# PolusAI/nyxus

Measured on AMD Instinct MI355X. Metric: ROIs/sec (*ALL_GLCM*+*ALL_INTENSITY*, 1024^2 tiles), higher is better.
Workload: dtype f64; 1 GPU; *ALL_GLCM*+*ALL_INTENSITY*, coarse_gray_depth=8, 4 angles, d=1, 1000 synthetic 1024x1024 tiles/GPU x 196 ROIs/tile (disk r=30, 2821 px, bbox 61x61), intensities U[1,4095]; reduce stage on pre-assembled ROI clouds resident in HBM; n_columns=185

## Files before the change

### nyxus_amd/csrc/roi_features.hip

```cpp
#include <hip/hip_runtime.h>
#include <type_traits>
#include <algorithm>
#include <cstdio>
#include "knobs.h"
#include "device_math.h"
#include "roi_kernel.h"
#include "launch_util.h"
#include "glcm_rows.h"
#include "glcm_w64.h"
#include "intensity_close.h"
#include "sort_lds.h"
#include "../../include/nyxhip.h"

namespace nyxhip {


enum { S_MEAN = 0, S_P10, S_P90, S_MEDIAN, S_MODE, S_NG, S_SLOPE };


template <int NW> __device__ __forceinline__ double xw_chain(const double* s_red, int k)
{
    return NW == 1 ? s_red[k] : ((s_red[k] + s_red[8 + k]) + s_red[16 + k]) + s_red[24 + k];
}
template <int NW> __device__ __forceinline__ double xw_pairs(const double* s_red, int k)
// ... 101 lines not shown
        for (int j = 0; j < Ng; j++, ic += (uint32_t)Ng) {
            cc += P[ic];
            rc += P[lN + (uint32_t)j];
        }
        uint32_t i1 = lN, i2 = (uint32_t)l;
#pragma unroll 1
        for (int x = l; x < Ng; x++, i1 += (uint32_t)Ng + 1u, i2 += (uint32_t)Ng + 1u) {
            dc += P[i1];
            if (l > 0)
                dc += P[i2];
        }
    }
    const uint32_t l1 = (uint32_t)l + 1u;
    const uint32_t csum = row16_sum(rc);
    const uint32_t Sr_i = row16_sum(mul24(rc, l1)), Sc_i = row16_sum(mul24(cc, l1));
    const uint32_t con_i = row16_sum(mul24(dc, (uint32_t)(l * l))), dis_i = row16_sum(mul24(dc, (uint32_t)l));
    const bool empty = csum == 0;
    const double sum_p = empty ? 1.0 : (double)csum;
    const double inv_sum_p = fdiv(1.0, sum_p);
    const double mr = fdiv((double)Sr_i, sum_p), mc = fdiv((double)Sc_i, sum_p);
    const double pcol = fdiv((double)cc, sum_p), prow = fdiv((double)rc, sum_p), pxmy = fdiv((double)dc, sum_p);
    if (live && l < Ng) { pcol_s[l] = pcol; prow_s[l] = prow; }
    for (int k = l; k < 2 * Ng - 1; k += 16) {
        uint32_t c = 0;
        const int x0 = k - (Ng - 1) > 0 ? k - (Ng - 1) : 0, x1 = k < Ng - 1 ? k : Ng - 1;
        uint32_t ix = mad24((uint32_t)x0, (uint32_t)Ng, (uint32_t)(k - x0));
#pragma unroll 1
        for (int x = x0; x <= x1; x++, ix += (uint32_t)Ng - 1u)
            c += P[ix];
        if (live) Pxpy[k] = fdiv((double)c, sum_p);
    }
    wav_sync<false>();

    double ent = 0, hxy1 = 0, hxy2 = 0, asm_d = 0;
    uint32_t acor_i = 0, asm_i = 0, cmax = 0;
    const bool big = csum >= 65536u;
    RowCol rcw((uint32_t)l, 16u, (uint32_t)Ng, RowCol::small_t{});
    for (int e = l; e < NN; e += 16, rcw.advance()) {
        const uint32_t r = rcw.row, c = rcw.col, cnt = P[e];
        const double p = (double)cnt * inv_sum_p;
        if (big) asm_d = __builtin_fma(p, p, asm_d);
        else asm_i = mad24(cnt, cnt, asm_i);
        acor_i = mad24(cnt, mul24(r + 1u, c + 1u), acor_i);
        cmax = cnt > cmax ? cnt : cmax;
        ent = __builtin_fma(p, (double)fast_log2f(p + 0.000000001), ent);
        const double pp = pcol_s[c] * prow_s[r];
        const double lg = (double)fast_log2f(pp + 0.000000001);
        hxy1 = __builtin_fma(p, lg, hxy1);
        hxy2 = __builtin_fma(pp, lg, hxy2);
    }
    const double hx_t = l < Ng ? plogp(pcol, pcol) : 0.0;
    {
        double t4[4] = {ent, hxy1, hxy2, hx_t};
        transpose_sum_step<0x140, 2>(t4, (l & 8) != 0);
        transpose_sum_step<0x141, 1>(t4, (l & 4) != 0);
        double tot = t4[0];
        tot += dpp_perm<0x4E>(tot);
        tot += dpp_perm<0xB1>(tot);
        if (live && (l & 3) == 0) sm[1 + (l >> 2)] = tot;
    }
    acor_i = row16_sum(acor_i);
    asm_i = row16_sum(asm_i);
    if (big) asm_d = row16_sum(asm_d);
    {
        uint32_t o;
        o = dpp_perm<0xB1>(cmax); cmax = o > cmax ? o : cmax;
        o = dpp_perm<0x4E>(cmax); cmax = o > cmax ? o : cmax;
        o = dpp_perm<0x141>(cmax); cmax = o > cmax ? o : cmax;
        o = dpp_perm<0x140>(cmax); cmax = o > cmax ? o : cmax;
    }

    double t16[16];
#pragma unroll
    for (int k = 0; k < 16; k++) t16[k] = 0.0;
    if (l < Ng) {
        const double dr = (double)l1 - mr, dcl = (double)l1 - mc, dr2 = dr * dr;
        t16[0] = prow * dr2;
        t16[1] = pcol * (dcl * dcl);
        t16[2] = (double)rc * dr2;
        t16[3] = pcol * dr2;
        const double q = pxmy, kd = (double)l, Ngd = (double)Ng;
        t16[4] = fdiv(q, (double)(1 + l * l));
        t16[5] = q != 0 ? plogp(q, q) : 0.0;
        t16[6] = fdiv(q, 1.0 + fdiv(kd * kd, Ngd * Ngd));
        t16[7] = fdiv(q, 1.0 + kd);
        t16[8] = fdiv(q, 1.0 + fdiv(kd, Ngd));
        t16[9] = l >= 1 ? q / (kd * kd) : 0.0;
        t16[10] = kd * q;
    }
    for (int k = l; k < 2 * Ng - 1; k += 16) {
        const double q = Pxpy[k], ks = (double)(k + 2);
        t16[11] += ks * q;
        t16[12] += plogp(q, q);
        const double m = ks - mc - mc, m2 = m * m;
        t16[13] += m2 * m2 * q;
        t16[14] += m2 * m * q;
        t16[15] += m2 * q;
    }
    {
        const double tot = row16_transpose_sum16(t16, l);
        if (live) sm[8 + l] = tot;
    }
    wav_sync<false>();
    const double davg = sm[8 + 10];
    double dv = 0;
    if (l < Ng) { const double dk = (double)l - davg; dv = dk * dk * pxmy; }
    dv = row16_sum(dv);

    if (live && l == 0) {
        const double ent_t = sm[1], hxy1_t = sm[2], hxy2_t = sm[3], hx = sm[4];
        const double asm_t = big ? asm_d : (double)asm_i * inv_sum_p * inv_sum_p;
        const double cov_t = ((double)acor_i * sum_p - (double)Sr_i * (double)Sc_i) * (inv_sum_p * inv_sum_p);
        f[G_ASM] = asm_t;
        f[G_ENERGY] = asm_t;
        f[G_CONTRAST] = (double)con_i * inv_sum_p;
        f[G_ACOR] = (double)acor_i * inv_sum_p;
        f[G_ENTROPY] = -ent_t;
        f[G_JE] = -ent_t;
        f[G_DIS] = (double)dis_i * inv_sum_p;
        f[G_JMAX] = (double)cmax * inv_sum_p;
        f[G_JAVE] = mr;
        f[G_VARIANCE] = sm[8 + 2] * inv_sum_p;
        f[G_CLUPROM] = sm[8 + 13];
        f[G_CLUSHADE] = sm[8 + 14];
        f[G_CLUTEND] = sm[8 + 15];
        f[G_SUMVARIANCE] = sm[8 + 15];
        f[G_JVAR] = sm[8 + 3];
        const double vv = sm[8 + 0] * sm[8 + 1];
        f[G_CORRELATION] = !(sm[8 + 0] > 0.0 && sm[8 + 1] > 0.0) ? soft_nan : cov_t * frsq(vv);
        f[G_INFOMEAS2] = sqrt(fabs(1 - exp(-2 * (-hxy2_t + ent_t))));
        f[G_IDM] = sm[8 + 4];
        f[G_HOM2] = sm[8 + 4];
        f[G_HOM1] = sm[8 + 7];
        f[G_SUMAVERAGE] = sm[8 + 11];
        f[G_SUMENTROPY] = -sm[8 + 12];
        f[G_DIFENTRO] = -sm[8 + 5];
        f[G_DIFAVE] = davg;
        f[G_DIFVAR] = dv;
        f[G_IDMN] = sm[8 + 6];
        f[G_ID] = sm[8 + 7];
        f[G_IDN] = sm[8 + 8];
        f[G_IV] = sm[8 + 9];
        const double r1 = (ent_t - hxy1_t) / hx;
        f[G_INFOMEAS1] = isfinite(r1) ? r1 : soft_nan;
        if (empty)
            for (int k = 0; k < kGlcmAngled; k++)
                f[k] = soft_nan;
    }
    wav_sync<false>();
}

__device__ __forceinline__ uint32_t grp8_sum(uint32_t v) { v += dpp_perm<0xB1>(v); v += dpp_perm<0x4E>(v); v += dpp_perm<0x141>(v); return v; }
__device__ __forceinline__ double grp8_sum(double v) { v += dpp_perm<0xB1>(v); v += dpp_perm<0x4E>(v); v += dpp_perm<0x141>(v); return v; }
__device__ __forceinline__ void glcm_features_wave8(const uint32_t* P_a, const uint32_t* P_b, int n_slots, int Ng_a, int Ng_b, double* scr_base, int scr_stride,
                                                    double soft_nan, double* fslots, size_t f_gap, double* sums, int lane)
{
    const int grp = lane >> 3, l = lane & 7, sel = grp >> 2, slot_raw = grp & 3;
    const int Ng = sel ? Ng_b : Ng_a;
    const int NN = Ng * Ng;
    const bool live = slot_raw < n_slots && Ng != 0;
    const int slot = slot_raw < n_slots ? slot_raw : 0;
    const uint32_t* P = (sel ? P_b : P_a) + mul24((uint32_t)slot, (uint32_t)NN);
    const int gslot = sel * kMaxAngles + slot;
    double* pcol_s = scr_base + mul24((uint32_t)gslot, (uint32_t)scr_stride);
    double* prow_s = pcol_s + 8;
    double* f = fslots + gslot * 32 + (sel ? f_gap : 0);
    double* sm = sums + gslot * 32;

    uint32_t cc = 0, rc = 0, dc = 0;
    if (l < Ng) {
        const uint32_t lN = mul24((uint32_t)l, (uint32_t)Ng);
        uint32_t ic = (uint32_t)l;
#pragma unroll 1
        for (int j = 0; j < Ng; j++, ic += (uint32_t)Ng) {
            cc += P[ic];
            rc += P[lN + (uint32_t)j];
        }
        uint32_t i1 = lN, i2 = (uint32_t)l;
#pragma unroll 1
        for (int x = l; x < Ng; x++, i1 += (uint32_t)Ng + 1u, i2 += (uint32_t)Ng + 1u) {
            dc += P[i1];
            if (l > 0) dc += P[i2];
        }
    }
    const uint32_t l1 = (uint32_t)l + 1u;
    const uint32_t csum = grp8_sum(rc);
    const uint32_t Sr_i = grp8_sum(mul24(rc, l1)), Sc_i = grp8_sum(mul24(cc, l1));
    const uint32_t con_i = grp8_sum(mul24(dc, (uint32_t)(l * l))), dis_i = grp8_sum(mul24(dc, (uint32_t)l));
    const bool empty = csum == 0;
    const double sum_p = empty ? 1.0 : (double)csum;
    const double inv_sum_p = fdiv(1.0, sum_p);
    const double mr = fdiv((double)Sr_i, sum_p), mc = fdiv((double)Sc_i, sum_p);
    const double pcol = fdiv((double)cc, sum_p), prow = fdiv((double)rc, sum_p), pxmy = fdiv((double)dc, sum_p);
    if (live && l < Ng) { pcol_s[l] = pcol; prow_s[l] = prow; }
    double pxpy[2] = {0.0, 0.0};
#pragma unroll
    for (int u = 0; u < 2; u++) {
        const int k = l + 8 * u;
        if (k < 2 * Ng - 1) {
            uint32_t c = 0;
            const int x0 = k - (Ng - 1) > 0 ? k - (Ng - 1) : 0, x1 = k < Ng - 1 ? k : Ng - 1;
            uint32_t ix = mad24((uint32_t)x0, (uint32_t)Ng, (uint32_t)(k - x0));
#pragma unroll 1
            for (int x = x0; x <= x1; x++, ix += (uint32_t)Ng - 1u) c += P[ix];
            pxpy[u] = fdiv((double)c, sum_p);
        }
    }
    wav_sync<false>();
#if defined(NYX_G8_EXIT) && NYX_G8_EXIT == 1
    if (live && l < Ng) f[l] = pcol + prow + pxmy + pxpy[0] + pxpy[1] + mr + mc + (double)(con_i + dis_i);
    return;
#endif

    double ent = 0, hxy1 = 0, hxy2 = 0, asm_d = 0;
    uint32_t acor_i = 0, asm_i = 0, cmax = 0;
    const bool big = csum >= 65536u;
    {
        RowCol rcw((uint32_t)l, 8u, (uint32_t)(Ng ? Ng : 1), RowCol::small_t{});
        for (int e = l; e < NN; e += 8, rcw.advance()) {
            const uint32_t r = rcw.row, c = rcw.col, cnt = P[e];
            const double p = (double)cnt * inv_sum_p;
            if (big) asm_d = __builtin_fma(p, p, asm_d);
            else asm_i = mad24(cnt, cnt, asm_i);
            acor_i = mad24(cnt, mul24(r + 1u, c + 1u), acor_i);
            cmax = cnt > cmax ? cnt : cmax;
            ent = __builtin_fma(p, (double)fast_log2f(p + 0.000000001), ent);
            const double pp = pcol_s[c] * prow_s[r];
            const double lg = (double)fast_log2f(pp + 0.000000001);
            hxy1 = __builtin_fma(p, lg, hxy1);
            hxy2 = __builtin_fma(pp, lg, hxy2);
        }
    }
#if defined(NYX_G8_EXIT) && NYX_G8_EXIT == 2
    if (live && l < Ng) f[l] = ent + hxy1 + hxy2 + asm_d + (double)(acor_i + asm_i + cmax);
    return;
#endif
    const double hx_t = l < Ng ? plogp(pcol, pcol) : 0.0;
    {
        double t4[4] = {ent, hxy1, hxy2, hx_t};
        transpose_sum_step<0x141, 2>(t4, (l & 4) != 0);
        transpose_sum_step<0x4E, 1>(t4, (l & 2) != 0);
        double tot = t4[0];
        tot += dpp_perm<0xB1>(tot);
        if (live && (l & 1) == 0) sm[1 + (l >> 1)] = tot;
    }
    acor_i = grp8_sum(acor_i);
    asm_i = grp8_sum(asm_i);
    if (big) asm_d = grp8_sum(asm_d);
    {
        uint32_t o;
        o = dpp_perm<0xB1>(cmax); cmax = o > cmax ? o : cmax;
        o = dpp_perm<0x4E>(cmax); cmax = o > cmax ? o : cmax;
        o = dpp_perm<0x141>(cmax); cmax = o > cmax ? o : cmax;
    }

    {
        double t8[8];
#pragma unroll
        for (int k = 0; k < 8; k++) t8[k] = 0.0;
        if (l < Ng) {
            const double dr = (double)l1 - mr, dcl = (double)l1 - mc, dr2 = dr * dr;
            t8[0] = prow * dr2;
            t8[1] = pcol * (dcl * dcl);
            t8[2] = (double)rc * dr2;
            t8[3] = pcol * dr2;
            const double q = pxmy, kd = (double)l, Ngd = (double)Ng;
            t8[4] = fdiv(q, (double)(1 + l * l));
            t8[5] = q != 0 ? plogp(q, q) : 0.0;
            t8[6] = fdiv(q, 1.0 + fdiv(kd * kd, Ngd * Ngd));
            t8[7] = fdiv(q, 1.0 + kd);
        }
        transpose_sum_step<0x141, 4>(t8, (l & 4) != 0);
        transpose_sum_step<0x4E, 2>(t8, (l & 2) != 0);
        transpose_sum_step<0xB1, 1>(t8, (l & 1) != 0);
        if (live) sm[8 + l] = t8[0];
    }
    {
        double t8[8];
#pragma unroll
        for (int k = 0; k < 8; k++) t8[k] = 0.0;
        if (l < Ng) {
            const double q = pxmy, kd = (double)l, Ngd = (double)Ng;
            t8[0] = fdiv(q, 1.0 + fdiv(kd, Ngd));
            t8[1] = l >= 1 ? q / (kd * kd) : 0.0;
            t8[2] = kd * q;
        }
#pragma unroll
        for (int u = 0; u < 2; u++) {
            const int k = l + 8 * u;
            if (k < 2 * Ng - 1) {
                const double q = pxpy[u], ks = (double)(k + 2);
                t8[3] += ks * q;
                t8[4] += plogp(q, q);
                const double m = ks - mc - mc, m2 = m * m;
                t8[5] += m2 * m2 * q;
                t8[6] += m2 * m * q;
                t8[7] += m2 * q;
            }
        }
        transpose_sum_step<0x141, 4>(t8, (l & 4) != 0);
        transpose_sum_step<0x4E, 2>(t8, (l & 2) != 0);
        transpose_sum_step<0xB1, 1>(t8, (l & 1) != 0);
        if (live) sm[16 + l] = t8[0];
    }
    wav_sync<false>();
#if defined(NYX_G8_EXIT) && NYX_G8_EXIT == 3
    return;
#endif
    const double davg = sm[8 + 10];
    double dv = 0;
    if (l < Ng) { const double dk = (double)l - davg; dv = dk * dk * pxmy; }
    dv = grp8_sum(dv);

    if (live && l == 0) {
        const double ent_t = sm[1], hxy1_t = sm[2], hxy2_t = sm[3], hx = sm[4];
        const double asm_t = big ? asm_d : (double)asm_i * inv_sum_p * inv_sum_p;
        const double cov_t = ((double)acor_i * sum_p - (double)Sr_i * (double)Sc_i) * (inv_sum_p * inv_sum_p);
        f[G_ASM] = asm_t;
        f[G_ENERGY] = asm_t;
        f[G_CONTRAST] = (double)con_i * inv_sum_p;
        f[G_ACOR] = (double)acor_i * inv_sum_p;
        f[G_ENTROPY] = -ent_t;
        f[G_JE] = -ent_t;
        f[G_DIS] = (double)dis_i * inv_sum_p;
        f[G_JMAX] = (double)cmax * inv_sum_p;
        f[G_JAVE] = mr;
        f[G_VARIANCE] = sm[8 + 2] * inv_sum_p;
        f[G_CLUPROM] = sm[8 + 13];
        f[G_CLUSHADE] = sm[8 + 14];
        f[G_CLUTEND] = sm[8 + 15];
        f[G_SUMVARIANCE] = sm[8 + 15];
        f[G_JVAR] = sm[8 + 3];
        const double vv = sm[8 + 0] * sm[8 + 1];
        f[G_CORRELATION] = !(sm[8 + 0] > 0.0 && sm[8 + 1] > 0.0) ? soft_nan : cov_t * frsq(vv);
        f[G_INFOMEAS2] = sqrt(fabs(1 - exp(-2 * (-hxy2_t + ent_t))));
        f[G_IDM] = sm[8 + 4];
        f[G_HOM2] = sm[8 + 4];
        f[G_HOM1] = sm[8 + 7];
        f[G_SUMAVERAGE] = sm[8 + 11];
        f[G_SUMENTROPY] = -sm[8 + 12];
        f[G_DIFENTRO] = -sm[8 + 5];
        f[G_DIFAVE] = davg;
        f[G_DIFVAR] = dv;
        f[G_IDMN] = sm[8 + 6];
        f[G_ID] = sm[8 + 7];
        f[G_IDN] = sm[8 + 8];
        f[G_IV] = sm[8 + 9];
        const double r1 = (ent_t - hxy1_t) / hx;
        f[G_INFOMEAS1] = isfinite(r1) ? r1 : soft_nan;
        if (empty)
            for (int k = 0; k < kGlcmAngled; k++) f[k] = soft_nan;
    }
    wav_sync<false>();
}

typedef unsigned short us2_t __attribute__((ext_vector_type(2)));
#ifdef NYX_G16_EXIT
#define G16_EXIT(k, keep) do { if ((k) == NYX_G16_EXIT) { ((double*)blk)[lane & 31] = (double)(keep); return; } } while (0)
#else
#define G16_EXIT(k, keep) do { } while (0)
#endif
template <int NG, int ROLE = 0>
__device__ __forceinline__ void glcm_features_wave64_v2(const uint16_t* P, int Ng_rt, uint32_t* blk, double soft_nan, int lane)
{
    const int Ng = NG ? NG : Ng_rt;
    typedef __attribute__((address_space(3))) const uint16_t lds_cu16_t;
    typedef __attribute__((address_space(3))) const uint32_t lds_cu32_t;
    typedef __attribute__((address_space(3))) uint32_t lds_u32_t;
    const int pitch = (Ng + 3) & ~1;
    double* const f = (double*)blk;
// ... 1924 lines not shown
                for (; a < na; a++)
                    init = init + s_f[a * 32 + k];
                o[kGlcmAngled * na + j] = na ? init / (double)na : 0.0;
            }
        }
    }

    STAMP(13);
    STAMP(14);
}

template <bool GS, bool C16, bool SPLIT, bool D8>
__global__ __launch_bounds__(kBlock, 4) void roi_features_kernel(const RoiArgs A)
{
    roi_features_body<GS, C16, SPLIT, D8>(A, blockIdx.x);
}

template <bool C16, bool SPLIT, bool D8>
__global__ __launch_bounds__(kBlock, 5) void roi_features_kernel_occ5(const RoiArgs A)
{
    roi_features_body<false, C16, SPLIT, D8, 0, 5>(A, blockIdx.x);
}
template <bool C16, bool SPLIT, bool D8>
__global__ __launch_bounds__(kBlock, 6) void roi_features_kernel_occ6(const RoiArgs A)
{
    roi_features_body<false, C16, SPLIT, D8, 0, 6>(A, blockIdx.x);
}
template <bool C16, bool SPLIT, bool D8>
__global__ __launch_bounds__(kBlock, 7) void roi_features_kernel_occ7(const RoiArgs A)
{
    roi_features_body<false, C16, SPLIT, D8, 0, 7>(A, blockIdx.x);
}
template <int FAM, int WIN>
__global__ __launch_bounds__(kBlock, 8) void roi_features_kernel_occ8(const RoiArgs A)
{
    roi_features_body<false, true, FAM == 1 || FAM == 3, true, FAM, 8, false, WIN, 4, FAM == 1 || FAM == 2>(A, (WIN == 1 && A.win.xcd_swz) ? xcd_slot(blockIdx.x, gridDim.x) : (uint64_t)blockIdx.x);
}
template <int FAM, int WIN>
__global__ __launch_bounds__(kBlock, 7) void roi_features_kernel_fam7(const RoiArgs A)
{
    roi_features_body<false, true, FAM == 1 || FAM == 3, true, FAM, 7, false, WIN>(A, (WIN == 1 && A.win.xcd_swz) ? xcd_slot(blockIdx.x, gridDim.x) : (uint64_t)blockIdx.x);
}
template <int FAM, int WIN>
__global__ __launch_bounds__(kBlock, 6) void roi_features_kernel_fam6(const RoiArgs A)
{
    roi_features_body<false, true, FAM == 1 || FAM == 3, true, FAM, 6, false, WIN>(A, (WIN == 1 && A.win.xcd_swz) ? xcd_slot(blockIdx.x, gridDim.x) : (uint64_t)blockIdx.x);
}

template <int WIN>
__global__ __launch_bounds__(kBlock, 4) void roi_features_kernel_g16(const RoiArgs A)
{
    roi_features_body<false, true, false, true, 0, 9, true, WIN>(A, (WIN == 1 && A.win.xcd_swz) ? xcd_slot(blockIdx.x, gridDim.x) : (uint64_t)blockIdx.x);
}

template <int WIN>
__global__ __launch_bounds__(512, 8) void roi_features_kernel_g16w8(const RoiArgs A)
{
    roi_features_body<false, true, false, true, 4, 9, true, WIN, 8>(A, (WIN == 1 && A.win.xcd_swz) ? xcd_slot(blockIdx.x, gridDim.x) : (uint64_t)blockIdx.x);
}

__device__ __forceinline__ bool glcm_roi_in_launch(const RoiArgs& A, uint64_t roi)
{
    if (A.sp.class_mask == 0) return true;
    return roi_in_launch(A.sp, (uint32_t)(A.px_offset[roi + 1] - A.px_offset[roi]), A.bbox_w[roi], A.bbox_h[roi], A.max_inten[roi] - A.min_inten[roi]);
}

__global__ __launch_bounds__(kBlock, 4) void glcm_features_kernel(const RoiArgs A)
{
    extern __shared__ __attribute__((aligned(16))) unsigned char lds_raw[];
    const int tid = threadIdx.x, lane = tid & 63, wave = __builtin_amdgcn_readfirstlane(tid >> 6);
    uint64_t roi;
    if (!roi_of_slot(A.sp, (uint64_t)blockIdx.x * kWaves + wave, A.n_roi, roi))
        return;
    const int Ng = glcm_roi_in_launch(A, roi) ? (int)A.glcm_ng[roi] : 0;
    if (Ng == 0)
        return;
    const int na = A.glcm_na, ngc = (int)A.L.ng_cap, NN = Ng * Ng;
    const size_t per_wave = (((size_t)4 * kMaxAngles * ngc * ngc + 15) & ~(size_t)15) + 8ull * (ngc + kMaxAngles * 6 * ngc + 2 * kMaxAngles * 32);
    unsigned char* base = lds_raw + (size_t)wave * per_wave;
    uint32_t* s_P = (uint32_t*)base;
    double* s_scr = (double*)(base + (((size_t)4 * kMaxAngles * ngc * ngc + 15) & ~(size_t)15)) + ngc;
    double* s_f = s_scr + kMaxAngles * 6 * ngc;
    const uint32_t* src = A.glcm_ws + roi * A.glcm_ws_stride;
    const int nw = na * NN;
    if (((nw | (int)A.glcm_ws_stride) & 3) == 0) {
#pragma unroll 1
        for (int i = lane; i < (nw >> 2); i += 64) ((uint4*)s_P)[i] = ((const uint4*)src)[i];
    } else {
#pragma unroll 1
        for (int i = lane; i < nw; i += 64) s_P[i] = src[i];
    }
    wav_sync<false>();
    glcm_features_wave16(s_P, na, Ng, s_scr, 6 * ngc, A.soft_nan, s_f, s_f + kMaxAngles * 32, lane);
    wav_sync<false>();
    double* o = A.out + roi * A.ld + A.col_glcm;
    const int sh = na == 4 ? 2 : na == 2 ? 1 : na == 1 ? 0 : -1;
    for (int c = lane; c < kGlcmAngled * na; c += 64) {
        const int k = sh >= 0 ? c >> sh : c / na, a = c - k * na;
        o[c] = s_f[a * 32 + k];
    }
    for (int j = lane; j < kGlcmAve; j += 64) {
        const int k = c_glcm_ave_order[j];
        double init = 0.0;
        int a = 0;
        for (; na - a >= 4; a += 4) {
            const double v1 = s_f[a * 32 + k] + s_f[(a + 1) * 32 + k];
            const double v2 = s_f[(a + 2) * 32 + k] + s_f[(a + 3) * 32 + k];
            init = init + (v1 + v2);
        }
        for (; a < na; a++)
            init = init + s_f[a * 32 + k];
        o[kGlcmAngled * na + j] = na == 4 ? init * 0.25 : na == 2 ? init * 0.5 : na ? init / (double)na : 0.0;
    }
}

__host__ __device__ inline size_t glcm8_cnt_bytes(uint32_t ngc)
{
    const size_t c = ((size_t)4 * kMaxAngles * ngc * ngc + 15) & ~(size_t)15, fbytes = 8ull * kMaxAngles * 32;
    return c > fbytes ? c : fbytes;
}
__global__ __launch_bounds__(kBlock, 8) void glcm_features_kernel8(const RoiArgs A)
{
    extern __shared__ __attribute__((aligned(16))) unsigned char lds_raw[];
    const int tid = threadIdx.x, lane = tid & 63, wave = __builtin_amdgcn_readfirstlane(tid >> 6);
    const uint64_t slot0 = ((uint64_t)blockIdx.x * kWaves + wave) * 2;
    uint64_t roi[2] = {0, 0};
    int Ng[2] = {0, 0};
#pragma unroll
    for (int q = 0; q < 2; q++)
        if (roi_of_slot(A.sp, slot0 + q, A.n_roi, roi[q]) && glcm_roi_in_launch(A, roi[q])) Ng[q] = (int)A.glcm_ng[roi[q]];
    if (Ng[0] == 0 && Ng[1] == 0)
        return;
    const int na = A.glcm_na, ngc = (int)A.L.ng_cap;
    const size_t cnt_bytes = glcm8_cnt_bytes((uint32_t)ngc);
    const size_t per_wave = 2 * cnt_bytes + 8ull * (2 * kMaxAngles * 16 + 2 * kMaxAngles * 32);
    unsigned char* base = lds_raw + (size_t)wave * per_wave;
    uint32_t* s_P[2] = {(uint32_t*)base, (uint32_t*)(base + cnt_bytes)};
    double* s_scr = (double*)(base + 2 * cnt_bytes);
    double* s_sum = s_scr + 2 * kMaxAngles * 16;
#pragma unroll
    for (int q = 0; q < 2; q++) {
        if (Ng[q] == 0) continue;
        const uint32_t* src = A.glcm_ws + roi[q] * A.glcm_ws_stride;
        const int nw = na * Ng[q] * Ng[q];
        if (((nw | (int)A.glcm_ws_stride) & 3) == 0) {
#pragma unroll 1
            for (int i = lane; i < (nw >> 2); i += 64) ((uint4*)s_P[q])[i] = ((const uint4*)src)[i];
        } else {
#pragma unroll 1
            for (int i = lane; i < nw; i += 64) s_P[q][i] = src[i];
        }
    }
    wav_sync<false>();
    glcm_features_wave8(s_P[0], s_P[1], na, Ng[0], Ng[1], s_scr, 16, A.soft_nan, (double*)base, (size_t)(cnt_bytes >> 3) - 4 * 32, s_sum, lane);
    wav_sync<false>();
    const int sh = na == 4 ? 2 : na == 2 ? 1 : na == 1 ? 0 : -1;
#pragma unroll
    for (int q = 0; q < 2; q++) {
        if (Ng[q] == 0) continue;
        double* o = A.out + roi[q] * A.ld + A.col_glcm;
        const double* fq = (const double*)(base + (size_t)q * cnt_bytes);
        for (int c = lane; c < kGlcmAngled * na; c += 64) {
            const int k = sh >= 0 ? c >> sh : c / na, a = c - k * na;
            o[c] = fq[a * 32 + k];
        }
        for (int j = lane; j < kGlcmAve; j += 64) {
            const int k = c_glcm_ave_order[j];
            double init = 0.0;
            int a = 0;
            for (; na - a >= 4; a += 4) {
                const double v1 = fq[a * 32 + k] + fq[(a + 1) * 32 + k];
                const double v2 = fq[(a + 2) * 32 + k] + fq[(a + 3) * 32 + k];
                init = init + (v1 + v2);
            }
            for (; a < na; a++) init = init + fq[a * 32 + k];
            o[kGlcmAngled * na + j] = na == 4 ? init * 0.25 : na == 2 ? init * 0.5 : na ? init / (double)na : 0.0;
        }
    }
}

constexpr int kCloseBlock = 64;
constexpr uint64_t kCloseCols =
    (1ull << I_MIN) | (1ull << I_MAX) | (1ull << I_RANGE) | (1ull << I_COVERED_IMAGE_INTENSITY_RANGE) | (1ull << I_MEAN) | (1ull << I_ENERGY) |
    (1ull << I_ROOT_MEAN_SQUARED) | (1ull << I_INTEGRATED_INTENSITY) | (1ull << I_UNIFORMITY_PIU) | (1ull << I_MEAN_ABSOLUTE_DEVIATION) |
    (1ull << I_VARIANCE) | (1ull << I_VARIANCE_BIASED) | (1ull << I_STANDARD_DEVIATION) | (1ull << I_STANDARD_DEVIATION_BIASED) | (1ull << I_COV) |
    (1ull << I_STANDARD_ERROR) | (1ull << I_SKEWNESS) | (1ull << I_KURTOSIS) | (1ull << I_EXCESS_KURTOSIS) | (1ull << I_HYPERSKEWNESS) |
    (1ull << I_HYPERFLATNESS) | (1ull << I_ROBUST_MEAN) | (1ull << I_MEDIAN_ABSOLUTE_DEVIATION) | (1ull << I_ROBUST_MEAN_ABSOLUTE_DEVIATION) |
    (1ull << I_QCOD) | (1ull << I_INTERQUARTILE_RANGE);
__global__ __launch_bounds__(kCloseBlock) void intensity_close_kernel(const RoiArgs A)
{
    constexpr int kPitch = __builtin_popcountll(kCloseCols);
#ifndef NYX_CLOSE_DIRECT
    __shared__ double s_o[kCloseBlock * kPitch];
#endif
    const int lane = (int)threadIdx.x;
    uint64_t roi = 0;
    bool mine = roi_of_slot(A.sp, (uint64_t)blockIdx.x * kCloseBlock + (uint64_t)lane, A.n_roi, roi) && glcm_roi_in_launch(A, roi);
    if (mine) mine = A.close_flag[roi] != 0;
    const unsigned long long todo = __ballot(mine);
    if (todo == 0)
        return;
#ifdef NYX_CLOSE_DIRECT
    double* const o = A.out + roi * A.ld + A.col_intensity;
    auto O = [&](int c) -> double& { return o[c]; };
#else
    double* const o = s_o + lane * kPitch;
    auto O = [&](int c) -> double& { return o[__builtin_popcountll(kCloseCols & ((1ull << c) - 1ull))]; };
#endif
    if (mine) {
        A.close_flag[roi] = 0;
        const double* const rec = A.close_rec + roi * kCloseRec;
        const uint32_t* const rw = (const uint32_t*)rec;
        const double* const row = A.out + roi * A.ld + A.col_intensity;
        const uint32_t n = (uint32_t)(A.px_offset[roi + 1] - A.px_offset[roi]);
        const uint32_t vmin = A.min_inten[roi], vmax = A.max_inten[roi];
        const double2 s01 = *(const double2*)(rec + CR_TOT);
        double acc[6];
#pragma unroll
        for (int k = 0; k < 6; k += 2) {
            const double2 t = *(const double2*)(rec + CR_ACC + k);
            acc[k] = t.x; acc[k + 1] = t.y;
        }
        const double sadk = rec[CR_SADK], adin0 = rec[CR_ADIN];
        const bool fast32 = rw[CR_W_FAST32] != 0;
        const uint4 w0 = *(const uint4*)(rw + CR_W_NBELOW), w1 = *(const uint4*)(rw + CR_W_LOX);
        const uint32_t n_below = w0.x, n_above = w0.y, K = w0.z, Sxu = w0.w, lox = w1.x, hix = w1.y, m2x = w1.z, cle = w1.w;
        const double p25 = row[I_P25], p75 = row[I_P75];
#pragma unroll
        for (int c = 0; c < kIntensityCols; c++)
            if ((kCloseCols >> c) & 1ull) O(c) = 0.0;
        const double dn = (double)n;
        constexpr bool blank = false;
        const double tot = s01.x, totsq = s01.y;
        const double mean = tot / dn;
        close_sums(O, dn, vmin, vmax, tot, totsq, mean, A.slide_min && A.slide_max, [&] { return A.slide_max[roi] - A.slide_min[roi]; }, blank);
        close_central<CovDiv::ieee>(O, acc, n, dn, mean, blank);
        const double Sx = (double)Sxu;
        close_robust_mad(O, sadk, m2x, cle, K, Sx, vmin, dn);
        close_robust_rmad(O, adin0, fast32, K, Sx, lox, hix, n_below, n_above);
        close_quartiles(O, p25, p75);
    }
#ifndef NYX_CLOSE_DIRECT
    __syncthreads();
    int mycol = -1;
    {
        int rank = 0;
#pragma unroll
        for (int c = 0; c < kIntensityCols; c++)
            if ((kCloseCols >> c) & 1ull) { if (rank == lane) mycol = c; rank++; }
    }
    double* const dst0 = A.out + A.col_intensity + (mycol >= 0 ? mycol : 0);
#pragma unroll 8
    for (int r = 0; r < kCloseBlock; r++) {
        if (!((todo >> r) & 1ull)) continue;
        const uint64_t rr = readlane_u64(roi, r);
        if (mycol >= 0)
            dst0[rr * A.ld] = s_o[r * kPitch + lane];
    }
#endif
}

size_t glcm_features8_lds(uint32_t ng_cap)
{
    return (2 * glcm8_cnt_bytes(ng_cap) + 8ull * (2 * kMaxAngles * 16 + 2 * kMaxAngles * 32)) * kWaves;
}

size_t glcm_features_lds(uint32_t ng_cap)
{
    const size_t per_wave = (((size_t)4 * kMaxAngles * ng_cap * ng_cap + 15) & ~(size_t)15) + 8ull * (ng_cap + kMaxAngles * 6 * ng_cap + 2 * kMaxAngles * 32);
    return per_wave * kWaves;
}

size_t roi_features_max_lds()
{
    return 160 * 1024;
}

namespace {

int no_static_lds(const void* f)
{
    hipFuncAttributes at;
    if (hipError_t e = hipFuncGetAttributes(&at, f); e != hipSuccess)
        return (int)e;
    return at.sharedSizeBytes == 0 ? 0 : (int)hipErrorInvalidConfiguration;
}

template <bool C16, bool SPLIT, bool D8>
int launch_lds_variant(const RoiArgs& a, hipStream_t st, uint32_t grid, bool& deferred)
{
    deferred = false;
    static DeviceOnce optin;
    if (int orc = optin.run([]() -> int {
        const void* fns[22] = {(const void*)roi_features_kernel<false, C16, SPLIT, D8>, (const void*)roi_features_kernel_occ5<C16, SPLIT, D8>,
                               (const void*)roi_features_kernel_occ6<C16, SPLIT, D8>, (const void*)roi_features_kernel_occ7<C16, SPLIT, D8>,
                               (const void*)roi_features_kernel_occ8<1, 0>, (const void*)roi_features_kernel_occ8<2, 0>,
                               (const void*)roi_features_kernel_occ8<1, 1>, (const void*)roi_features_kernel_occ8<2, 1>,
                               (const void*)roi_features_kernel_fam7<1, 0>, (const void*)roi_features_kernel_fam7<2, 0>,
                               (const void*)roi_features_kernel_fam7<1, 1>, (const void*)roi_features_kernel_fam7<2, 1>,
                               (const void*)roi_features_kernel_fam6<1, 0>, (const void*)roi_features_kernel_fam6<2, 0>,
                               (const void*)roi_features_kernel_fam6<1, 1>, (const void*)roi_features_kernel_fam6<2, 1>,
                               (const void*)roi_features_kernel_occ8<3, 0>, (const void*)roi_features_kernel_occ8<3, 1>,
                               (const void*)roi_features_kernel_fam7<3, 0>, (const void*)roi_features_kernel_fam7<3, 1>,
                               (const void*)roi_features_kernel_fam6<3, 0>, (const void*)roi_features_kernel_fam6<3, 1>};
        for (const void* f : fns) {
            hipError_t e = hipFuncSetAttribute(f, hipFuncAttributeMaxDynamicSharedMemorySize, (int)roi_features_max_lds());
            if (e != hipSuccess)
// ... 118 lines not shown
```

Baseline: 113.0 million ROIs/s.

## Add Ng=8, four-angle specialised GLCM feature path with unrolled marginals

Adds a template specialisation of the wave8 GLCM feature routine, used when four angles are present and both ROIs have Ng of 0 or 8. Row, column, diagonal-difference and anti-diagonal sums are computed by fully unrolled, per-lane strided loads with mask-based wrap selection and DPP shuffles, replacing variable-trip loops. The main entropy/correlation loop becomes a fixed 8-iteration unrolled column walk that reuses the lane's own pcol and no longer needs RowCol index tracking. The general path remains for other shapes, at the cost of extra code size and register pressure.

```diff
diff --git a/nyxus_amd/csrc/roi_features.hip b/nyxus_amd/csrc/roi_features.hip
--- a/nyxus_amd/csrc/roi_features.hip
+++ b/nyxus_amd/csrc/roi_features.hip
@@ -277,13 +277,59 @@
 
 __device__ __forceinline__ uint32_t grp8_sum(uint32_t v) { v += dpp_perm<0xB1>(v); v += dpp_perm<0x4E>(v); v += dpp_perm<0x141>(v); return v; }
 __device__ __forceinline__ double grp8_sum(double v) { v += dpp_perm<0xB1>(v); v += dpp_perm<0x4E>(v); v += dpp_perm<0x141>(v); return v; }
+__device__ __forceinline__ bool lanes_l_above(int x)
+{
+    return __builtin_amdgcn_inverse_ballot_w64(((0xFFull << (x + 1)) & 0xFFull) * 0x0101010101010101ull);
+}
+__device__ __forceinline__ bool lanes_l_below(int x)
+{
+    return __builtin_amdgcn_inverse_ballot_w64(((1ull << x) - 1ull) * 0x0101010101010101ull);
+}
+__device__ __forceinline__ void glcm_marginal_counts_o8(const uint32_t* P, int l, uint32_t& cc, uint32_t& rc, uint32_t& dc, uint32_t (&ac)[2])
+{
+    cc = 0;
+#pragma unroll
+    for (int u = 0; u < 8; u++) cc += P[8 * u + l];
+    const uint4 r0 = ((const uint4*)(P + 8 * l))[0], r1 = ((const uint4*)(P + 8 * l))[1];
+    rc = ((r0.x + r0.y) + (r0.z + r0.w)) + ((r1.x + r1.y) + (r1.z + r1.w));
+    const uint32_t* d_lo = P + 9 - l;
+    const uint32_t* d_hi = d_lo + 8;
+    const uint32_t d0 = P[(8 - l) & 7];
+    uint32_t tot = d0, up = lanes_l_above(0) ? d0 : 0u;
+#pragma unroll
+    for (int x = 1; x < 8; x++) {
+        const bool wrap = x < 7 && lanes_l_above(x);
+        const uint32_t d = (wrap ? d_hi : d_lo)[9 * (x - 1)];
+        tot += d;
+        if (x < 7) up += wrap ? d : 0u;
+    }
+    dc = (tot - up) + dpp_perm<0x111>(dpp_perm<0x141>(up));
+    const uint32_t* a_lo = P + l;
+    const uint32_t* a_hi = a_lo + 8;
+    uint32_t atot = 0, ahi = 0;
+#pragma unroll
+    for (int x = 0; x < 8; x++) {
+        const bool wrap = x > 0 && lanes_l_below(x);
+        const uint32_t a = (wrap ? a_hi : a_lo)[7 * x];
+        atot += a;
+        if (x > 0) ahi += wrap ? a : 0u;
+    }
+    ac[0] = atot - ahi;
+    ac[1] = ahi;
+}
+
+#ifndef NYX_G8_O8_PARTS
+#define NYX_G8_O8_PARTS 3
+#endif
+template <bool O8>
 __device__ __forceinline__ void glcm_features_wave8(const uint32_t* P_a, const uint32_t* P_b, int n_slots, int Ng_a, int Ng_b, double* scr_base, int scr_stride,
                                                     double soft_nan, double* fslots, size_t f_gap, double* sums, int lane)
 {
+    constexpr bool O8M = O8 && (NYX_G8_O8_PARTS & 1), O8C = O8 && (NYX_G8_O8_PARTS & 2);
     const int grp = lane >> 3, l = lane & 7, sel = grp >> 2, slot_raw = grp & 3;
-    const int Ng = sel ? Ng_b : Ng_a;
+    const int Ng_roi = sel ? Ng_b : Ng_a, Ng = O8 ? 8 : Ng_roi;
     const int NN = Ng * Ng;
-    const bool live = slot_raw < n_slots && Ng != 0;
+    const bool live = slot_raw < n_slots && Ng_roi != 0;
     const int slot = slot_raw < n_slots ? slot_raw : 0;
     const uint32_t* P = (sel ? P_b : P_a) + mul24((uint32_t)slot, (uint32_t)NN);
     const int gslot = sel * kMaxAngles + slot;
@@ -293,7 +339,10 @@
     double* sm = sums + gslot * 32;
 
     uint32_t cc = 0, rc = 0, dc = 0;
-    if (l < Ng) {
+    uint32_t ac8[2];
+    if constexpr (O8M) {
+        glcm_marginal_counts_o8(P, l, cc, rc, dc, ac8);
+    } else if (l < Ng) {
         const uint32_t lN = mul24((uint32_t)l, (uint32_t)Ng);
         uint32_t ic = (uint32_t)l;
 #pragma unroll 1
@@ -324,10 +373,14 @@
         const int k = l + 8 * u;
         if (k < 2 * Ng - 1) {
             uint32_t c = 0;
-            const int x0 = k - (Ng - 1) > 0 ? k - (Ng - 1) : 0, x1 = k < Ng - 1 ? k : Ng - 1;
-            uint32_t ix = mad24((uint32_t)x0, (uint32_t)Ng, (uint32_t)(k - x0));
+            if constexpr (O8M) {
+                c = ac8[u];
+            } else {
+                const int x0 = k - (Ng - 1) > 0 ? k - (Ng - 1) : 0, x1 = k < Ng - 1 ? k : Ng - 1;
+                uint32_t ix = mad24((uint32_t)x0, (uint32_t)Ng, (uint32_t)(k - x0));
 #pragma unroll 1
-            for (int x = x0; x <= x1; x++, ix += (uint32_t)Ng - 1u) c += P[ix];
+                for (int x = x0; x <= x1; x++, ix += (uint32_t)Ng - 1u) c += P[ix];
+            }
             pxpy[u] = fdiv((double)c, sum_p);
         }
     }
@@ -340,7 +393,32 @@
     double ent = 0, hxy1 = 0, hxy2 = 0, asm_d = 0;
     uint32_t acor_i = 0, asm_i = 0, cmax = 0;
     const bool big = csum >= 65536u;
-    {
+    if constexpr (O8C) {
+        const uint32_t* Pl = P + l;
+        if (big) {
+#pragma unroll
+            for (int u = 0; u < 8; u++) {
+                const double p = (double)Pl[8 * u] * inv_sum_p;
+                asm_d = __builtin_fma(p, p, asm_d);
+            }
+        }
+        uint32_t wgt = l1;
+#pragma unroll
+        for (int u = 0; u < 8; u++) {
+            const uint32_t cnt = Pl[8 * u];
+            const double p = (double)cnt * inv_sum_p;
+            asm_i = mad24(cnt, cnt, asm_i);
+            acor_i = mad24(cnt, wgt, acor_i);
+            wgt += l1;
+            cmax = cnt > cmax ? cnt : cmax;
+            ent = __builtin_fma(p, (double)fast_log2f(p + 0.000000001), ent);
+            const double pp = pcol * prow_s[u];
+            const double lg = (double)fast_log2f(pp + 0.000000001);
+            hxy1 = __builtin_fma(p, lg, hxy1);
+            hxy2 = __builtin_fma(pp, lg, hxy2);
+            __builtin_amdgcn_sched_barrier(0);
+        }
+    } else {
         RowCol rcw((uint32_t)l, 8u, (uint32_t)(Ng ? Ng : 1), RowCol::small_t{});
         for (int e = l; e < NN; e += 8, rcw.advance()) {
             const uint32_t r = rcw.row, c = rcw.col, cnt = P[e];
@@ -2571,7 +2649,10 @@
         }
     }
     wav_sync<false>();
-    glcm_features_wave8(s_P[0], s_P[1], na, Ng[0], Ng[1], s_scr, 16, A.soft_nan, (double*)base, (size_t)(cnt_bytes >> 3) - 4 * 32, s_sum, lane);
+    if (na != 4 || ((Ng[0] | Ng[1]) & ~8) != 0)
+        glcm_features_wave8<false>(s_P[0], s_P[1], na, Ng[0], Ng[1], s_scr, 16, A.soft_nan, (double*)base, (size_t)(cnt_bytes >> 3) - 4 * 32, s_sum, lane);
+    else
+        glcm_features_wave8<true>(s_P[0], s_P[1], 4, Ng[0], Ng[1], s_scr, 16, A.soft_nan, (double*)base, (size_t)(cnt_bytes >> 3) - 4 * 32, s_sum, lane);
     wav_sync<false>();
     const int sh = na == 4 ? 2 : na == 2 ? 1 : na == 1 ? 0 : -1;
 #pragma unroll
```

Measured after the change: 116.4 million ROIs/s, median of 6. 1.03x the previous value.
